# rensortino/DDP-Tutorial

Hardware: AMD Instinct MI355X
Metric: images/sec (whole node), ResNet-18 CIFAR-10 (higher is better)
Workload: dtype bf16; 1 GPU; model=resnet18, global_batch=8192, image_size=32, num_classes=10, parallelism=dp1, sync_bn=False, hip_graph=False

## Files before the change

mi355x/csrc/bindings.cpp:

```cpp
#include <torch/extension.h>

#include <tuple>
#include <vector>

at::Tensor relu_bwd(at::Tensor dy, at::Tensor y);
at::Tensor mfma_probe32(at::Tensor A, at::Tensor B);
void sgd_step(at::Tensor p, at::Tensor g, at::Tensor m, double lr, double mu,
              double wd, double gscale);
void grad_stats(at::Tensor g, at::Tensor slab, at::Tensor out);
void sgd_step_guarded(at::Tensor p, at::Tensor g, at::Tensor m,
                      at::Tensor state, c10::optional<at::Tensor> lr_dev,
                      double lr, double mu, double wd, double gscale,
                      double max_norm, c10::optional<at::Tensor> ema,
                      c10::optional<at::Tensor> clock);
void clock_advance(at::Tensor clock, c10::optional<at::Tensor> state,
                   at::Tensor table, double decay, bool warmup);
void scaler_update(at::Tensor state, double gscale, double max_norm,
                   double growth, double backoff, long interval);
void lars_stats(at::Tensor p, at::Tensor g, at::Tensor table, at::Tensor tens,
                at::Tensor slab, at::Tensor state, at::Tensor stats,
                double gscale, double max_norm, double wd, double eta,
                double eps);
void lars_step(at::Tensor p, at::Tensor g, at::Tensor m, at::Tensor table,
               at::Tensor tens, at::Tensor state, at::Tensor stats,
               c10::optional<at::Tensor> lr_dev, double lr, double mu,
               double wd, double gscale, double max_norm,
               c10::optional<at::Tensor> ema, c10::optional<at::Tensor> clock);
at::Tensor cast_to_16(at::Tensor src, at::Tensor like);
at::Tensor cast_permute_krsc(at::Tensor w, at::Tensor like);
at::Tensor cast_permute_krsc_pad(at::Tensor w, at::Tensor like);
at::Tensor cast_permute_rsck(at::Tensor w, at::Tensor like);

at::Tensor conv2d_fwd(at::Tensor x, at::Tensor w, at::Tensor bias,
                      long stride, long pad, long act, long kR, long kS);
at::Tensor conv2d_dgrad(at::Tensor dy, at::Tensor wflip, long stride,
                        long pad, long H, long W, at::Tensor addin);
at::Tensor conv2d_wgrad(at::Tensor x, at::Tensor dy, long R, long S,
                        long stride, long pad);
std::vector<at::Tensor> conv2d_fwd_stats(at::Tensor x, at::Tensor w,
                                         long stride, long pad, long kR,
                                         long kS);
std::vector<at::Tensor> conv2d_fwd_scaled(at::Tensor x, at::Tensor w,
                                          at::Tensor asc, at::Tensor ash,
                                          long stride, long pad,
                                          bool want_stats);
at::Tensor conv2d_wgrad_scaled(at::Tensor x, at::Tensor asc, at::Tensor ash,
                               at::Tensor dy, long R, long S, long stride,
                               long pad);

at::Tensor bn_stats(at::Tensor x);
at::Tensor bn_finalize(at::Tensor stats, at::Tensor running_mean,
                       at::Tensor running_var, double m_total,
                       double momentum, double eps);
std::vector<at::Tensor> bn_apply(at::Tensor x, at::Tensor mean, at::Tensor invstd,
                    at::Tensor gamma, at::Tensor beta, at::Tensor res,
                    long act, bool want_mask);
at::Tensor bn_bwd_reduce(at::Tensor x, at::Tensor dy, at::Tensor y,
                         at::Tensor mean, at::Tensor invstd,
                         at::Tensor mask, at::Tensor asc, at::Tensor ash);
std::vector<at::Tensor> bn_bwd_dx(at::Tensor x, at::Tensor dy, at::Tensor y,
                                  at::Tensor mean, at::Tensor invstd,
                                  at::Tensor gamma, at::Tensor dgamma,
                                  at::Tensor dbeta, double m_total,
                                  bool want_dres, at::Tensor mask,
                                  at::Tensor asc, at::Tensor ash);

std::vector<at::Tensor> maxpool_fwd(at::Tensor x, long kernel, long stride,
                                    long pad);
at::Tensor maxpool_bwd(at::Tensor dy, at::Tensor idx, long H, long W,
                       long kernel, long stride, long pad);
at::Tensor global_avg_pool(at::Tensor x);

at::Tensor linear_fwd(at::Tensor x, at::Tensor w, at::Tensor bias, long act);
at::Tensor linear_dgrad(at::Tensor dy, at::Tensor w, at::Tensor wt);
at::Tensor linear_wgrad(at::Tensor x, at::Tensor dy);
at::Tensor gemm_nt_mfma(at::Tensor A, at::Tensor B, at::Tensor bias, long act,
                        bool out32);

std::vector<at::Tensor> cross_entropy_fwd(at::Tensor logits,
                                          at::Tensor target);
at::Tensor cross_entropy_bwd(at::Tensor logits, at::Tensor target,
                             at::Tensor lse, at::Tensor dloss);
std::vector<at::Tensor> cross_entropy_soft_fwd(
    at::Tensor logits, at::Tensor y_a, c10::optional<at::Tensor> y_b,
    c10::optional<at::Tensor> lam, double eps);
at::Tensor cross_entropy_soft_bwd(at::Tensor logits, at::Tensor y_a,
                                  c10::optional<at::Tensor> y_b,
                                  c10::optional<at::Tensor> lam,
                                  at::Tensor lse, at::Tensor dloss,
                                  double eps);
void meter_update(at::Tensor state, at::Tensor slab, at::Tensor logits,
                  at::Tensor y_a, c10::optional<at::Tensor> y_b,
                  c10::optional<at::Tensor> lam, long k,
                  c10::optional<at::Tensor> loss,
                  c10::optional<at::Tensor> confusion, long pack);

std::tuple<at::Tensor, at::Tensor> gather_augment(
    at::Tensor data_u8, at::Tensor targets, at::Tensor indices,
    at::Tensor scale, at::Tensor shift, int64_t pad, bool flip, int64_t seed,
    int64_t epoch, at::Tensor like);
std::tuple<at::Tensor, at::Tensor, at::Tensor, at::Tensor> gather_augment_mix(
    at::Tensor data_u8, at::Tensor targets, at::Tensor indices,
    at::Tensor scale, at::Tensor shift, int64_t pad, bool flip, int64_t tc,
    int64_t tm, double inv_hw, int64_t seed, int64_t epoch, at::Tensor like);

void register_rccl(py::module_& m);

PYBIND11_MODULE(TORCH_EXTENSION_NAME, m) {
  register_rccl(m);
  m.def("relu_bwd", &relu_bwd);
  m.def("mfma_probe32", &mfma_probe32);
  m.def("sgd_step", &sgd_step);
  m.def("grad_stats", &grad_stats);
  m.def("sgd_step_guarded", &sgd_step_guarded);
  m.def("scaler_update", &scaler_update);
  m.def("clock_advance", &clock_advance);
  m.def("lars_stats", &lars_stats);
  m.def("lars_step", &lars_step);
  m.def("cast_to_16", &cast_to_16);
  m.def("cast_permute_krsc", &cast_permute_krsc);
  m.def("cast_permute_krsc_pad", &cast_permute_krsc_pad);
  m.def("cast_permute_rsck", &cast_permute_rsck);
  m.def("conv2d_fwd", &conv2d_fwd);
  m.def("conv2d_dgrad", &conv2d_dgrad);
  m.def("conv2d_wgrad", &conv2d_wgrad);
  m.def("conv2d_fwd_stats", &conv2d_fwd_stats);
  m.def("conv2d_fwd_scaled", &conv2d_fwd_scaled);
  m.def("conv2d_wgrad_scaled", &conv2d_wgrad_scaled);
  m.def("bn_stats", &bn_stats);
  m.def("bn_finalize", &bn_finalize);
  m.def("bn_apply", &bn_apply);
  m.def("bn_bwd_reduce", &bn_bwd_reduce);
  m.def("bn_bwd_dx", &bn_bwd_dx);
  m.def("maxpool_fwd", &maxpool_fwd);
  m.def("maxpool_bwd", &maxpool_bwd);
  m.def("global_avg_pool", &global_avg_pool);
  m.def("linear_fwd", &linear_fwd);
  m.def("linear_dgrad", &linear_dgrad);
  m.def("linear_wgrad", &linear_wgrad);
  m.def("gemm_nt_mfma", &gemm_nt_mfma);
  m.def("cross_entropy_fwd", &cross_entropy_fwd);
  m.def("cross_entropy_bwd", &cross_entropy_bwd);
  m.def("cross_entropy_soft_fwd", &cross_entropy_soft_fwd);
  m.def("cross_entropy_soft_bwd", &cross_entropy_soft_bwd);
  m.def("meter_update", &meter_update);
  m.def("gather_augment", &gather_augment);
  m.def("gather_augment_mix", &gather_augment_mix);
}
```

mi355x/csrc/bn.hip:

```cpp
#include "common.h"

namespace {

template <typename T16>
__global__ void bn_stats_kernel(const T16* __restrict__ x,
                                float* __restrict__ out,
                                long M, int C, long m_per_chunk) {
  const int c = blockIdx.y * blockDim.x + threadIdx.x;
  if (c >= C) return;
  const long m0 = (long)blockIdx.x * m_per_chunk;
  const long m1 = min(M, m0 + m_per_chunk);
  float s = 0.f, ss = 0.f;
  for (long m = m0; m < m1; ++m) {
    const float v = F16<T16>::to_f32(x[m * C + c]);
    s += v;
    ss += v * v;
  }
  float* o = out + (long)blockIdx.x * 2 * C;
  o[c] = s;
  o[C + c] = ss;
}

template <typename T16>
__global__ void bn_apply_kernel(const T16* __restrict__ x,
// ... 162 lines not shown
__global__ __launch_bounds__(256) void bn_apply_fast(
    const T16* __restrict__ x, const float* __restrict__ mean,
    const float* __restrict__ invstd, const float* __restrict__ gamma,
    const float* __restrict__ beta, const T16* __restrict__ res,
    T16* __restrict__ y, unsigned char* __restrict__ msk, long E, int C,
    int act) {
  const int c0 = ((blockIdx.x * blockDim.x + threadIdx.x) * 8) % C;
  float sc[8], sh[8];
#pragma unroll
  for (int u = 0; u < 8; ++u) {
    sc[u] = gamma[c0 + u] * invstd[c0 + u];
    sh[u] = beta[c0 + u] - mean[c0 + u] * sc[u];
  }
  const long stride = (long)gridDim.x * blockDim.x * 8;
  auto body = [&](long e) {
    const short8 vx = *reinterpret_cast<const short8*>(x + e);
    short8 vr = {};
    if (res) vr = *reinterpret_cast<const short8*>(res + e);
    short8 o;
    unsigned mb = 0;
#pragma unroll
    for (int u = 0; u < 8; ++u) {
      float v = s16_to_f32<T16>(vx[u]) * sc[u] + sh[u];
      if (res) v += s16_to_f32<T16>(vr[u]);
      if (act == 1) v = relu_f(v);
      o[u] = f32_to_s16<T16>(v);
      if (s16_to_f32<T16>(o[u]) > 0.f) mb |= 1u << u;
    }
    *reinterpret_cast<short8*>(y + e) = o;
    if (msk) msk[e >> 3] = (unsigned char)mb;
  };
  long e = (long)(blockIdx.x * blockDim.x + threadIdx.x) * 8;
  for (; e + stride < E; e += 2 * stride) {
    body(e);
    body(e + stride);
  }
  for (; e < E; e += stride) body(e);
}

template <typename T16, bool RC = false>
__global__ __launch_bounds__(256) void bn_bwd_dx_fast(
    const T16* __restrict__ x, const T16* __restrict__ dy,
    const unsigned char* __restrict__ msk, const float* __restrict__ mean,
    const float* __restrict__ invstd, const float* __restrict__ gamma,
    const float* __restrict__ dgamma, const float* __restrict__ dbeta,
    const float* __restrict__ asc, const float* __restrict__ ash,
    T16* __restrict__ dx, T16* __restrict__ dres, long E, int C,
    float inv_m) {
  const int c0 = ((blockIdx.x * blockDim.x + threadIdx.x) * 8) % C;
  float mu[8], is[8], g_[8], a_[8], b_[8], ac[8], ah[8];
#pragma unroll
  for (int u = 0; u < 8; ++u) {
    mu[u] = mean[c0 + u];
    is[u] = invstd[c0 + u];
    g_[u] = gamma[c0 + u] * is[u];
    a_[u] = dgamma[c0 + u] * inv_m;
    b_[u] = dbeta[c0 + u] * inv_m;
    if (RC) {
      ac[u] = asc[c0 + u];
      ah[u] = ash[c0 + u];
    }
  }
  const long stride = (long)gridDim.x * blockDim.x * 8;
  auto body = [&](long e) {
    const short8 vx = *reinterpret_cast<const short8*>(x + e);
    const short8 vd = *reinterpret_cast<const short8*>(dy + e);
    const unsigned mb = msk ? msk[e >> 3] : 0xffu;
    short8 odx, ods;
#pragma unroll
    for (int u = 0; u < 8; ++u) {
      float d = s16_to_f32<T16>(vd[u]);
      const float xv = s16_to_f32<T16>(vx[u]);
      if (RC) {
        if (xv * ac[u] + ah[u] <= 0.f) d = 0.f;
      } else if (!((mb >> u) & 1)) {
        d = 0.f;
      }
      if (dres) ods[u] = f32_to_s16<T16>(d);
      const float xh = (xv - mu[u]) * is[u];
      odx[u] = f32_to_s16<T16>(g_[u] * (d - b_[u] - xh * a_[u]));
    }
    *reinterpret_cast<short8*>(dx + e) = odx;
    if (dres) *reinterpret_cast<short8*>(dres + e) = ods;
  };
  long e = (long)(blockIdx.x * blockDim.x + threadIdx.x) * 8;
  for (; e + stride < E; e += 2 * stride) {
    body(e);
    body(e + stride);
  }
  for (; e < E; e += stride) body(e);
}

__global__ void bn_finalize_kernel(const float* __restrict__ stats,
                                   float* __restrict__ out,
                                   float* __restrict__ rmean,
                                   float* __restrict__ rvar, int C,
                                   float inv_m, float unbias, float momentum,
                                   float eps) {
  const int c = blockIdx.x * blockDim.x + threadIdx.x;
  if (c >= C) return;
  const float mean = stats[c] * inv_m;
  const float var = stats[C + c] * inv_m - mean * mean;
  out[c] = mean;
  out[C + c] = rsqrtf(var + eps);
  if (rmean) {
    rmean[c] = rmean[c] * (1.f - momentum) + mean * momentum;
    rvar[c] = rvar[c] * (1.f - momentum) + var * unbias * momentum;
  }
}

inline bool bn_fast_ok(long M, int C) {
  return C % 8 == 0 && 2048 % C == 0;
}

inline size_t bn_reduce_lds(int C) {
  const int rows = C > 512 ? 4 / (C / 512) : 4;
  return sizeof(float) * rows * 2 * C;
}

inline at::Tensor bn_partial_rows(const at::Tensor& x, unsigned nrows, int C) {
  return at::empty({(long)nrows, 2, C}, x.options().dtype(at::kFloat));
}

inline at::Tensor bn_fold(at::Tensor part, unsigned nrows, int C) {
  if (nrows == 1) return part.view({2, C});
  auto out = at::empty({2, C}, part.options());
  fold_rows(part, out, 2L * C, nrows);
  return out;
}

inline dim3 bn_fast_grid(long E, long& e_per_block) {
  static const long cap = EnvKnob("MI355X_BN_BLOCKS").num(512);
  long blocks = std::min<long>(cdiv_l(E, 2048), cap);
  e_per_block = cdiv_l(cdiv_l(E, blocks), 2048) * 2048;
  blocks = cdiv_l(E, e_per_block);
  return dim3((unsigned)blocks);
}

inline dim3 chan_grid(long M, int C, long& m_per_chunk, int block = 256) {
  const int cblocks = cdiv_i(C, block);
  long chunks = std::min<long>(cdiv_l(M, 1024), std::max(1, 2048 / cblocks));
  chunks = std::max<long>(chunks, 1);
  m_per_chunk = cdiv_l(M, chunks);
  return dim3((unsigned)chunks, cblocks);
}

inline int ew_grid2(long n, int block = 256) {
  return (int)std::min<long>(cdiv_l(n, block), 4096);
}

}

at::Tensor bn_finalize(at::Tensor stats, at::Tensor running_mean,
                       at::Tensor running_var, double m_total,
                       double momentum, double eps) {
  const int C = stats.size(1);
  auto out = at::empty_like(stats);
  const bool has_run = running_mean.numel() > 0;
  const double unbias = m_total / std::max(m_total - 1.0, 1.0);
  hipLaunchKernelGGL(bn_finalize_kernel, dim3(cdiv_i(C, 256)), dim3(256), 0,
                     cur_stream(), stats.data_ptr<float>(),
                     out.data_ptr<float>(),
                     has_run ? running_mean.data_ptr<float>() : nullptr,
                     has_run ? running_var.data_ptr<float>() : nullptr, C,
                     (float)(1.0 / m_total), (float)unbias, (float)momentum,
                     (float)eps);
// ... 105 lines not shown
                           mask.numel() ? mask.data_ptr<unsigned char>()
                                        : nullptr,
                           mean.data_ptr<float>(), invstd.data_ptr<float>(),
                           nullptr, nullptr,
                           out.data_ptr<float>(), E, C, e_per_block);
    });
    return bn_fold(out, grid.x, C);
  }
  long m_per_chunk;
  dim3 grid = chan_grid(M, C, m_per_chunk);
  auto out = bn_partial_rows(x, grid.x, C);
  DISPATCH_16(x, T16, {
    hipLaunchKernelGGL(bn_bwd_reduce_kernel<T16>, grid, dim3(256), 0,
                       cur_stream(), (const T16*)x.data_ptr(),
                       (const T16*)dy.data_ptr(),
                       y.numel() ? (const T16*)y.data_ptr() : nullptr,
                       mean.data_ptr<float>(),
                       invstd.data_ptr<float>(), out.data_ptr<float>(), M, C,
                       m_per_chunk);
  });
  return bn_fold(out, grid.x, C);
}

std::vector<at::Tensor> bn_bwd_dx(at::Tensor x, at::Tensor dy, at::Tensor y,
                                  at::Tensor mean, at::Tensor invstd,
                                  at::Tensor gamma, at::Tensor dgamma,
                                  at::Tensor dbeta, double m_total,
                                  bool want_dres, at::Tensor mask,
                                  at::Tensor asc, at::Tensor ash) {
  TORCH_CHECK(!(asc.defined() && asc.numel() > 0) ||
                  bn_fast_ok(x.numel() / x.size(-1), x.size(-1)),
              "mask recompute (asc/ash) needs the fast BN path");
  CHECK_GPU(x);
  CHECK_CONTIG(dy);
  const int C = x.size(-1);
  const long M = x.numel() / C;
  auto dx = at::empty_like(x);
  auto dres = want_dres ? at::empty_like(x) : at::Tensor();
  if (bn_fast_ok(M, C)) {
    const long E = M * (long)C;
    const int grid = (int)std::min<long>(cdiv_l(E, 256 * 8), 2048);
    const bool rc = asc.defined() && asc.numel() > 0;
    DISPATCH_16(x, T16, {
      if (rc)
        hipLaunchKernelGGL((bn_bwd_dx_fast<T16, true>), dim3(grid),
                           dim3(256), 0, cur_stream(),
                           (const T16*)x.data_ptr(),
                           (const T16*)dy.data_ptr(), nullptr,
                           mean.data_ptr<float>(), invstd.data_ptr<float>(),
                           gamma.data_ptr<float>(), dgamma.data_ptr<float>(),
                           dbeta.data_ptr<float>(), asc.data_ptr<float>(),
                           ash.data_ptr<float>(), (T16*)dx.data_ptr(),
                           want_dres ? (T16*)dres.data_ptr() : nullptr, E, C,
                           (float)(1.0 / m_total));
      else
        hipLaunchKernelGGL((bn_bwd_dx_fast<T16>), dim3(grid), dim3(256), 0,
                           cur_stream(), (const T16*)x.data_ptr(),
                           (const T16*)dy.data_ptr(),
                           mask.numel() ? mask.data_ptr<unsigned char>()
                                        : nullptr,
                           mean.data_ptr<float>(), invstd.data_ptr<float>(),
                           gamma.data_ptr<float>(), dgamma.data_ptr<float>(),
                           dbeta.data_ptr<float>(), nullptr, nullptr,
                           (T16*)dx.data_ptr(),
                           want_dres ? (T16*)dres.data_ptr() : nullptr, E, C,
                           (float)(1.0 / m_total));
    });
    return {dx, want_dres ? dres : at::Tensor()};
  }
  DISPATCH_16(x, T16, {
    hipLaunchKernelGGL(bn_bwd_dx_kernel<T16>, dim3(ew_grid2(M * C)),
                       dim3(256), 0, cur_stream(), (const T16*)x.data_ptr(),
                       (const T16*)dy.data_ptr(),
                       y.numel() ? (const T16*)y.data_ptr() : nullptr,
                       mean.data_ptr<float>(),
                       invstd.data_ptr<float>(), gamma.data_ptr<float>(),
                       dgamma.data_ptr<float>(), dbeta.data_ptr<float>(),
                       (T16*)dx.data_ptr(),
                       want_dres ? (T16*)dres.data_ptr() : nullptr, M, C,
                       (float)(1.0 / m_total));
  });
  return {dx, want_dres ? dres : at::Tensor()};
}
```

mi355x/models/layers.py:

```python

from __future__ import annotations

import math
import os

import torch
from torch import nn

from mi355x import ops


def to_model_layout(x: torch.Tensor) -> torch.Tensor:
    x = x.permute(0, 2, 3, 1)
    if x.is_cuda:
        x = x.to(ops.compute_dtype())
    return x.contiguous()


class Conv2d(nn.Module):

    def __init__(self, in_channels, out_channels, kernel_size, stride=1,
                 padding=0, bias=True, act=None, groups=1):
        super().__init__()
        if groups < 1 or in_channels % groups or out_channels % groups:
# ... 30 lines not shown
    def reset_parameters(self):
        nn.init.kaiming_uniform_(self.weight, a=math.sqrt(5))
        if self.bias is not None:
            bound = 1 / math.sqrt(self.weight.shape[1])
            nn.init.uniform_(self.bias, -bound, bound)

    def forward(self, x):
        return ops.linear(x, self.weight, self.bias, self.act)


class BatchNorm2d(nn.Module):

    def __init__(self, num_features, momentum=0.1, act=None):
        super().__init__()
        self.momentum, self.act = momentum, act
        self.weight = nn.Parameter(torch.ones(num_features))
        self.bias = nn.Parameter(torch.zeros(num_features))
        self.register_buffer("running_mean", torch.zeros(num_features))
        self.register_buffer("running_var", torch.ones(num_features))
        self._nbt = 0
        self.process_group = None

    @property
    def num_batches_tracked(self):
        return torch.tensor(self._nbt, dtype=torch.long)

    @num_batches_tracked.setter
    def num_batches_tracked(self, v):
        self._nbt = int(v)

    def _save_to_state_dict(self, destination, prefix, keep_vars):
        super()._save_to_state_dict(destination, prefix, keep_vars)
        destination[prefix + "num_batches_tracked"] = torch.tensor(
            self._nbt, dtype=torch.long)

    def _load_from_state_dict(self, state_dict, prefix, local_metadata,
                              strict, missing_keys, unexpected_keys,
                              error_msgs):
        key = prefix + "num_batches_tracked"
        if key in state_dict:
            self._nbt = int(state_dict[key])
        super()._load_from_state_dict(state_dict, prefix, local_metadata,
                                      strict, missing_keys, unexpected_keys,
                                      error_msgs)
        if key in unexpected_keys:
            unexpected_keys.remove(key)

    def forward(self, x, residual=None, stats=None):
        if self.training:
            self._nbt += 1
        return ops.batch_norm(x, self.weight, self.bias, self.running_mean,
                              self.running_var, self.training, self.momentum,
                              residual, self.act,
                              self.process_group if self.training else None,
                              stats)


def _fuse_stats():
    return os.environ.get("MI355X_FUSE_BN", "1") == "1"


def conv_bn(conv: "Conv2d", bn: "BatchNorm2d", x, residual=None):
    if (_fuse_stats() and x.is_cuda and bn.training and conv.bias is None
            and conv.act is None
            and (conv.weight.shape[1] % 64 == 0
                 or (conv.weight.shape[1] == 3
                     and ((conv.weight.shape[2] == 7 and conv.stride == 2)
                          or (conv.weight.shape[2] == 3
                              and conv.stride == 1))))):
        from mi355x.ops import functional as F_

        bn._nbt += 1

        y, stats = F_.conv2d_with_stats(x, conv.weight, conv.stride,
                                        conv.padding)
        if stats.numel() == 0:
            stats = None
        return ops.batch_norm(y, bn.weight, bn.bias, bn.running_mean,
                              bn.running_var, bn.training, bn.momentum,
                              residual, bn.act, bn.process_group, stats)
    return bn(conv(x), residual=residual)


def _tap_on():
    return os.environ.get("MI355X_TAP", "1") != "0"


def _lazy_mode():
    return os.environ.get("MI355X_LAZY_BN", "0")


def _lazy_ok(bn: "BatchNorm2d", conv: "Conv2d", x) -> bool:
    mode = _lazy_mode()
    if mode == "0":
        return False
    if mode == "g" and conv.weight.shape[2] != 1 and conv.stride == 1:
        return False
    C = conv.weight.shape[1]
    return (x.is_cuda and bn.training and bn.act == "relu"
            and conv.bias is None and conv.act is None
            and C % 64 == 0 and conv.weight.shape[0] % 64 == 0
            and 2048 % C == 0)


def bn_then_conv(bn: "BatchNorm2d", conv: "Conv2d", x, stats=None,
                 want_stats=False):
    if _lazy_ok(bn, conv, x) and x.requires_grad:
        return bn_conv_lazy(bn, conv, x, stats, want_stats)
    z = bn(x, stats=stats)
    if (want_stats and _fuse_stats() and z.is_cuda and bn.training
            and conv.bias is None and conv.act is None
            and conv.weight.shape[1] % 64 == 0):
        from mi355x.ops import functional as F_

        y, s2 = F_.conv2d_with_stats(z, conv.weight, conv.stride,
                                     conv.padding)
        if s2 is not None and s2.numel() == 0:
            s2 = None
        return y, s2
    return conv(z), None


def bn_conv_lazy(bn: "BatchNorm2d", conv: "Conv2d", x, stats=None,
                 want_stats=False):
    from mi355x.ops import functional as F_

    if bn.training:
        bn._nbt += 1
    out = F_.bn_conv(x, bn.weight, bn.bias, conv.weight, bn.running_mean,
                     bn.running_var, bn.momentum, stats,
                     bn.process_group if bn.training else None,
                     conv.stride, conv.padding, want_stats)
    if want_stats:
        y, s2 = out
        return y, (s2 if s2 is not None and s2.numel() else None)
    return out, None


def conv_bn_tap(conv: "Conv2d", bn: "BatchNorm2d", x, residual=None):
    if not (_tap_on() and x.is_cuda and conv.bias is None
            and conv.act is None):
        return conv_bn(conv, bn, x, residual=residual), x
    from mi355x.ops import functional as F_

    if _fuse_stats() and bn.training and conv.weight.shape[1] % 64 == 0:
        y, tap, stats = F_.conv2d_tap_stats(x, conv.weight, conv.stride,
                                            conv.padding)
        return bn(y, residual=residual, stats=stats), tap
    y, tap = F_.conv2d_tap(x, conv.weight, conv.stride, conv.padding)
    return bn(y, residual=residual), tap


class MaxPool2d(nn.Module):
    def __init__(self, kernel_size, stride=None, padding=0):
        super().__init__()
        self.kernel_size = kernel_size
        self.stride = stride or kernel_size
        self.padding = padding

    def forward(self, x):
        return ops.max_pool2d(x, self.kernel_size, self.stride, self.padding)
```

mi355x/models/resnet.py:

```python

from __future__ import annotations

import torch
from torch import nn

from .layers import (BatchNorm2d, Conv2d, Linear, MaxPool2d, _lazy_ok,
                     bn_conv_lazy, bn_then_conv, conv_bn, conv_bn_tap,
                     to_model_layout)
from mi355x import ops


class BasicBlock(nn.Module):
    expansion = 1

    def __init__(self, in_planes, planes, stride=1, downsample=None):
        super().__init__()
        self.conv1 = Conv2d(in_planes, planes, 3, stride, 1, bias=False)
        self.bn1 = BatchNorm2d(planes, act="relu")
        self.conv2 = Conv2d(planes, planes, 3, 1, 1, bias=False)
        self.bn2 = BatchNorm2d(planes, act="relu")
        self.downsample = downsample

    def forward(self, x):
        if _lazy_ok(self.bn1, self.conv2, x) and x.requires_grad:
            from mi355x.ops import functional as F_

            y1, tap, stats1 = F_.conv2d_tap_stats(
                x, self.conv1.weight, self.conv1.stride, self.conv1.padding)
            identity = (tap if self.downsample is None
                        else self.downsample(tap))
            y2, stats2 = bn_conv_lazy(self.bn1, self.conv2, y1, stats1,
                                      want_stats=True)
            return self.bn2(y2, residual=identity, stats=stats2)
        out, tap = conv_bn_tap(self.conv1, self.bn1, x)
        identity = tap if self.downsample is None else self.downsample(tap)
        out = conv_bn(self.conv2, self.bn2, out, residual=identity)
        return out


class Bottleneck(nn.Module):
    expansion = 4

    def __init__(self, in_planes, planes, stride=1, downsample=None):
        super().__init__()
        self.conv1 = Conv2d(in_planes, planes, 1, bias=False)
        self.bn1 = BatchNorm2d(planes, act="relu")
        self.conv2 = Conv2d(planes, planes, 3, stride, 1, bias=False)
        self.bn2 = BatchNorm2d(planes, act="relu")
        self.conv3 = Conv2d(planes, planes * 4, 1, bias=False)
        self.bn3 = BatchNorm2d(planes * 4, act="relu")
        self.downsample = downsample

    def forward(self, x):
        if x.is_cuda and x.requires_grad and self.bn1.training and (
                _lazy_ok(self.bn1, self.conv2, x)
                or _lazy_ok(self.bn2, self.conv3, x)):
            from mi355x.ops import functional as F_

            y1, tap, stats1 = F_.conv2d_tap_stats(
                x, self.conv1.weight, self.conv1.stride, self.conv1.padding)
            identity = (tap if self.downsample is None
                        else self.downsample(tap))
            y2, stats2 = bn_then_conv(self.bn1, self.conv2, y1, stats1,
                                      want_stats=True)
            y3, stats3 = bn_then_conv(self.bn2, self.conv3, y2, stats2,
                                      want_stats=True)
            return self.bn3(y3, residual=identity, stats=stats3)
        out, tap = conv_bn_tap(self.conv1, self.bn1, x)
        identity = tap if self.downsample is None else self.downsample(tap)
        out = conv_bn(self.conv2, self.bn2, out)
        out = conv_bn(self.conv3, self.bn3, out, residual=identity)
        return out


class Downsample(nn.Module):
    def __init__(self, in_planes, out_planes, stride):
        super().__init__()
        self.conv = Conv2d(in_planes, out_planes, 1, stride, bias=False)
        self.bn = BatchNorm2d(out_planes)

    def forward(self, x):
        return conv_bn(self.conv, self.bn, x)


class ResNet(nn.Module):
    def __init__(self, block, layers, num_classes=10, stem="cifar"):
        super().__init__()
        self.in_planes = 64
        if stem == "cifar":
            self.conv1 = Conv2d(3, 64, 3, 1, 1, bias=False)
            self.maxpool = None
        else:
            self.conv1 = Conv2d(3, 64, 7, 2, 3, bias=False)
            self.maxpool = MaxPool2d(3, 2, 1)
        self.bn1 = BatchNorm2d(64, act="relu")
        self.layer1 = self._make_layer(block, 64, layers[0], 1)
        self.layer2 = self._make_layer(block, 128, layers[1], 2)
        self.layer3 = self._make_layer(block, 256, layers[2], 2)
        self.layer4 = self._make_layer(block, 512, layers[3], 2)
        self.fc = Linear(512 * block.expansion, num_classes)
        for m in self.modules():
            if isinstance(m, Conv2d):
                nn.init.kaiming_normal_(m.weight, mode="fan_out",
                                        nonlinearity="relu")

    def _make_layer(self, block, planes, blocks, stride):
        downsample = None
        if stride != 1 or self.in_planes != planes * block.expansion:
            downsample = Downsample(self.in_planes, planes * block.expansion,
                                    stride)
        layers = [block(self.in_planes, planes, stride, downsample)]
        self.in_planes = planes * block.expansion
        layers += [block(self.in_planes, planes) for _ in range(1, blocks)]
        return nn.Sequential(*layers)

    def forward(self, x):
        x = to_model_layout(x)
        x = conv_bn(self.conv1, self.bn1, x)
        if self.maxpool is not None:
            x = self.maxpool(x)
        x = self.layer1(x)
        x = self.layer2(x)
        x = self.layer3(x)
        x = self.layer4(x)
        x = ops.global_avg_pool(x)
        return self.fc(x)


def resnet18(num_classes=10, stem="cifar"):
    return ResNet(BasicBlock, [2, 2, 2, 2], num_classes, stem)


def resnet50(num_classes=1000, stem="imagenet"):
    return ResNet(Bottleneck, [3, 4, 6, 3], num_classes, stem)
```

mi355x/ops/functional.py:

```python

from __future__ import annotations

from typing import NamedTuple

import numpy as np
import torch
import torch.nn.functional as F

from ._ext import ext

BN_EPS = 1e-5

_ACT_NONE = 0
_ACT_RELU = 1


def compute_dtype() -> torch.dtype:
    from mi355x import amp

    return amp.get_compute_dtype()



_cache_epoch = 0
# ... 325 lines not shown
        ctx.conf = (act, bias is not None)
        return y

    @staticmethod
    def backward(ctx, dy):
        x, w16, y = ctx.saved_tensors
        act, has_bias = ctx.conf
        dy = dy.contiguous()
        if act == _ACT_RELU:
            dy = _relu_mask_bwd(dy, y)
        dx = None
        if ctx.needs_input_grad[0]:
            wt = _w16_linear_t(ctx.weight_ref, dy.dtype)
            dx = ext().linear_dgrad(dy, w16, wt)
        dw = ext().linear_wgrad(x, dy) if ctx.needs_input_grad[1] else None
        db = dy.float().sum(dim=0) if (has_bias and ctx.needs_input_grad[2]) else None
        return dx, dw, db, None


def linear(x, weight, bias=None, act=None):
    a = _ACT_RELU if act == "relu" else _ACT_NONE
    if x.is_cuda:
        return _LinearFn.apply(x, weight, bias, a)
    y = F.linear(x, weight, bias)
    if a == _ACT_RELU:
        y = F.relu(y)
    return y




class _BNFn(torch.autograd.Function):

    @staticmethod
    def forward(ctx, x, gamma, beta, residual, running_mean, running_var,
                momentum, act, process_group, stats=None):
        N, H, W, C = x.shape
        m_local = N * H * W
        s = stats if stats is not None else ext().bn_stats(x)
        m_total = m_local
        if process_group is not None:
            import torch.distributed as dist

            dist.all_reduce(s, group=process_group)
            m_total = m_local * dist.get_world_size(process_group)
        empty = torch.empty(0, device=x.device)
        mi = ext().bn_finalize(
            s, running_mean if running_mean is not None else empty,
            running_var if running_var is not None else empty,
            float(m_total), momentum, BN_EPS)
        mean, invstd = mi[0], mi[1]
        res = residual if residual is not None else torch.empty(0, device=x.device, dtype=x.dtype)
        y, mask = ext().bn_apply(x, mean, invstd, gamma.detach().float(),
                                 beta.detach().float(), res, act, True)
        if mask is None:
            mask = torch.empty(0, device=x.device, dtype=torch.uint8)
        ctx.save_for_backward(x, y, mean, invstd, gamma, mask)
        ctx.conf = (act, residual is not None, m_total, process_group)
        return y

    @staticmethod
    def backward(ctx, dy):
        x, y, mean, invstd, gamma, mask = ctx.saved_tensors
        act, has_res, m_total, pg = ctx.conf
        dy = dy.contiguous()
        y_arg = y if act == _ACT_RELU else torch.empty(0, device=x.device,
                                                       dtype=x.dtype)
        ef = torch.empty(0, device=x.device)
        r = ext().bn_bwd_reduce(x, dy, y_arg, mean, invstd, mask, ef, ef)
        if pg is not None:
            import torch.distributed as dist

            dist.all_reduce(r, group=pg)
        dgamma, dbeta = r[0], r[1]
        want_dres = has_res and act == _ACT_RELU
        dx, dres = ext().bn_bwd_dx(x, dy, y_arg, mean, invstd,
                                   gamma.detach().float(), dgamma, dbeta,
                                   float(m_total), want_dres, mask, ef, ef)
        if has_res and not want_dres:
            dres = dy
        elif not has_res:
            dres = None
        return dx, dgamma, dbeta, dres, None, None, None, None, None, None


def batch_norm(x, gamma, beta, running_mean, running_var, training,
               momentum=0.1, residual=None, act=None, process_group=None,
               stats=None):
    a = _ACT_RELU if act == "relu" else _ACT_NONE
    if x.is_cuda:
        if training:
            return _BNFn.apply(x, gamma, beta, residual, running_mean,
                               running_var, momentum, a, process_group,
                               stats)
        mean = running_mean.float()
        invstd = torch.rsqrt(running_var.float() + BN_EPS)
        res = residual if residual is not None else torch.empty(0, device=x.device, dtype=x.dtype)
        return ext().bn_apply(x.contiguous(), mean, invstd,
                              gamma.detach().float(), beta.detach().float(),
                              res, a, False)[0]
    xc = x.permute(0, 3, 1, 2)
    y = F.batch_norm(xc, running_mean, running_var, gamma, beta, training,
                     momentum, BN_EPS).permute(0, 2, 3, 1)
    if residual is not None:
        y = y + residual
    if a == _ACT_RELU:
        y = F.relu(y)
    return y




class _MaxPoolFn(torch.autograd.Function):
    @staticmethod
    def forward(ctx, x, kernel, stride, padding):
        y, idx = ext().maxpool_fwd(x, kernel, stride, padding)
        ctx.save_for_backward(idx)
        ctx.conf = (x.shape, kernel, stride, padding)
        return y

    @staticmethod
    def backward(ctx, dy):
        (idx,) = ctx.saved_tensors
        xshape, kernel, stride, padding = ctx.conf
        dx = ext().maxpool_bwd(dy.contiguous(), idx, xshape[1], xshape[2],
                               kernel, stride, padding)
        return dx, None, None, None


def max_pool2d(x, kernel, stride=None, padding=0):
    stride = stride or kernel
    if x.is_cuda:
        return _MaxPoolFn.apply(x, kernel, stride, padding)
    y = F.max_pool2d(x.permute(0, 3, 1, 2), kernel, stride, padding)
    return y.permute(0, 2, 3, 1)


class _GAPFn(torch.autograd.Function):
    @staticmethod
    def forward(ctx, x):
        ctx.conf = x.shape
        return ext().global_avg_pool(x)

    @staticmethod
    def backward(ctx, dy):
        N, H, W, C = ctx.conf
        dx = (dy / (H * W)).reshape(N, 1, 1, C).expand(N, H, W, C).contiguous()
        return dx


def global_avg_pool(x):
    if x.is_cuda:
        return _GAPFn.apply(x)
    return x.mean(dim=(1, 2))




class _CEFn(torch.autograd.Function):
    @staticmethod
    def forward(ctx, logits, target):
        loss, lse = ext().cross_entropy_fwd(logits, target)
        ctx.save_for_backward(logits, target, lse)
        return loss

    @staticmethod
# ... 520 lines not shown
```

Baseline: 157,500 images/sec.

## Fuse downsample BN with main-branch BN, residual add and ReLU in one pass

Adds dual batch-norm kernels that normalize both the main conv output and the downsample conv output, add them, apply ReLU and emit a bit mask in one elementwise pass. The backward pass computes both branches' reductions and input gradients in shared passes. The goal is to avoid materializing the normalized downsample tensor and to cut separate full-tensor read/write passes in the three downsample blocks of ResNet-18. It is on by default, gated by an env flag, and relies on the fused-stats conv path and a specific channel layout.

```diff
diff --git a/mi355x/csrc/bindings.cpp b/mi355x/csrc/bindings.cpp
--- a/mi355x/csrc/bindings.cpp
+++ b/mi355x/csrc/bindings.cpp
@@ -64,6 +64,21 @@
                                   at::Tensor dbeta, double m_total,
                                   bool want_dres, at::Tensor mask,
                                   at::Tensor asc, at::Tensor ash);
+std::vector<at::Tensor> bn_apply_dual(at::Tensor x, at::Tensor mean,
+                                      at::Tensor invstd, at::Tensor gamma,
+                                      at::Tensor beta, at::Tensor xr,
+                                      at::Tensor mean_r, at::Tensor invstd_r,
+                                      at::Tensor gamma_r, at::Tensor beta_r);
+at::Tensor bn_bwd_reduce_dual(at::Tensor x, at::Tensor xr, at::Tensor dy,
+                              at::Tensor mask, at::Tensor mean,
+                              at::Tensor invstd, at::Tensor mean_r,
+                              at::Tensor invstd_r);
+std::vector<at::Tensor> bn_bwd_dx_dual(at::Tensor x, at::Tensor xr,
+                                       at::Tensor dy, at::Tensor mask,
+                                       at::Tensor mean, at::Tensor invstd,
+                                       at::Tensor gamma, at::Tensor mean_r,
+                                       at::Tensor invstd_r, at::Tensor gamma_r,
+                                       at::Tensor red, double m_total);
 
 std::vector<at::Tensor> maxpool_fwd(at::Tensor x, long kernel, long stride,
                                     long pad);
@@ -132,6 +147,9 @@
   m.def("bn_apply", &bn_apply);
   m.def("bn_bwd_reduce", &bn_bwd_reduce);
   m.def("bn_bwd_dx", &bn_bwd_dx);
+  m.def("bn_apply_dual", &bn_apply_dual);
+  m.def("bn_bwd_reduce_dual", &bn_bwd_reduce_dual);
+  m.def("bn_bwd_dx_dual", &bn_bwd_dx_dual);
   m.def("maxpool_fwd", &maxpool_fwd);
   m.def("maxpool_bwd", &maxpool_bwd);
   m.def("global_avg_pool", &global_avg_pool);
diff --git a/mi355x/csrc/bn.hip b/mi355x/csrc/bn.hip
--- a/mi355x/csrc/bn.hip
+++ b/mi355x/csrc/bn.hip
@@ -268,6 +268,176 @@
     }
     *reinterpret_cast<short8*>(dx + e) = odx;
     if (dres) *reinterpret_cast<short8*>(dres + e) = ods;
+  };
+  long e = (long)(blockIdx.x * blockDim.x + threadIdx.x) * 8;
+  for (; e + stride < E; e += 2 * stride) {
+    body(e);
+    body(e + stride);
+  }
+  for (; e < E; e += stride) body(e);
+}
+
+template <typename T16>
+__global__ __launch_bounds__(256) void bn_apply_dual_fast(
+    const T16* __restrict__ x, const T16* __restrict__ xr,
+    const float* __restrict__ mean, const float* __restrict__ invstd,
+    const float* __restrict__ gamma, const float* __restrict__ beta,
+    const float* __restrict__ mean_r, const float* __restrict__ invstd_r,
+    const float* __restrict__ gamma_r, const float* __restrict__ beta_r,
+    T16* __restrict__ y, unsigned char* __restrict__ msk, long E, int C) {
+  const int c0 = ((blockIdx.x * blockDim.x + threadIdx.x) * 8) % C;
+  float sc[8], sh[8], scr[8], shr[8];
+#pragma unroll
+  for (int u = 0; u < 8; ++u) {
+    sc[u] = gamma[c0 + u] * invstd[c0 + u];
+    sh[u] = beta[c0 + u] - mean[c0 + u] * sc[u];
+    scr[u] = gamma_r[c0 + u] * invstd_r[c0 + u];
+    shr[u] = beta_r[c0 + u] - mean_r[c0 + u] * scr[u];
+  }
+  const long stride = (long)gridDim.x * blockDim.x * 8;
+  auto body = [&](long e) {
+    const short8 vx = *reinterpret_cast<const short8*>(x + e);
+    const short8 vr = *reinterpret_cast<const short8*>(xr + e);
+    short8 o;
+    unsigned mb = 0;
+#pragma unroll
+    for (int u = 0; u < 8; ++u) {
+      float rf = s16_to_f32<T16>(vr[u]) * scr[u] + shr[u];
+      asm("" : "+v"(rf));
+      const float r = s16_to_f32<T16>(f32_to_s16<T16>(rf));
+      float v = s16_to_f32<T16>(vx[u]) * sc[u] + sh[u];
+      v += r;
+      v = relu_f(v);
+      o[u] = f32_to_s16<T16>(v);
+      if (s16_to_f32<T16>(o[u]) > 0.f) mb |= 1u << u;
+    }
+    *reinterpret_cast<short8*>(y + e) = o;
+    msk[e >> 3] = (unsigned char)mb;
+  };
+  long e = (long)(blockIdx.x * blockDim.x + threadIdx.x) * 8;
+  for (; e + stride < E; e += 2 * stride) {
+    body(e);
+    body(e + stride);
+  }
+  for (; e < E; e += stride) body(e);
+}
+
+template <typename T16>
+__global__ __launch_bounds__(256) void bn_reduce_dual_fast(
+    const T16* __restrict__ x, const T16* __restrict__ xr,
+    const T16* __restrict__ dy, const unsigned char* __restrict__ msk,
+    const float* __restrict__ mean, const float* __restrict__ invstd,
+    const float* __restrict__ mean_r, const float* __restrict__ invstd_r,
+    float* __restrict__ out,
+    long E, int C, long e_per_block) {
+  extern __shared__ __attribute__((aligned(16))) float lsum[];
+  const int tid = threadIdx.x;
+  const int c0 = (tid * 8) % C;
+  float s0[8] = {}, sr[8] = {}, s1[8] = {};
+  float mu[8], is[8], mur[8], isr[8];
+#pragma unroll
+  for (int u = 0; u < 8; ++u) {
+    mu[u] = mean[c0 + u];
+    is[u] = invstd[c0 + u];
+    mur[u] = mean_r[c0 + u];
+    isr[u] = invstd_r[c0 + u];
+  }
+  const long e0 = (long)blockIdx.x * e_per_block;
+  const long e1 = min(E, e0 + e_per_block);
+  constexpr long ESTEP = 256 * 8;
+  auto body = [&](long e) {
+    const short8 vx = *reinterpret_cast<const short8*>(x + e);
+    const short8 vr = *reinterpret_cast<const short8*>(xr + e);
+    const short8 vd = *reinterpret_cast<const short8*>(dy + e);
+    const unsigned mb = msk[e >> 3];
+#pragma unroll
+    for (int u = 0; u < 8; ++u) {
+      float d = s16_to_f32<T16>(vd[u]);
+      if (!((mb >> u) & 1)) d = 0.f;
+      const float xh = (s16_to_f32<T16>(vx[u]) - mu[u]) * is[u];
+      const float xhr = (s16_to_f32<T16>(vr[u]) - mur[u]) * isr[u];
+      s0[u] += d * xh;
+      sr[u] += d * xhr;
+      s1[u] += d;
+    }
+  };
+  long e = e0 + (long)tid * 8;
+  for (; e + 3 * ESTEP < e1; e += 4 * ESTEP) {
+#pragma unroll
+    for (int v = 0; v < 4; ++v) body(e + v * ESTEP);
+  }
+  for (; e < e1; e += ESTEP) body(e);
+  const int gstride = C / 8;
+  for (int off = 32; off >= gstride && off >= 1; off >>= 1) {
+#pragma unroll
+    for (int u = 0; u < 8; ++u) {
+      s0[u] += __shfl_xor(s0[u], off, kWave);
+      sr[u] += __shfl_xor(sr[u], off, kWave);
+      s1[u] += __shfl_xor(s1[u], off, kWave);
+    }
+  }
+  const bool leader = (threadIdx.x & 63) < gstride || gstride >= 64;
+  const int wpr = C > 512 ? C / 512 : 1;
+  const int rows = 4 / wpr;
+  const int row = (tid >> 6) / wpr;
+  if (leader) {
+#pragma unroll
+    for (int u = 0; u < 8; ++u) {
+      lsum[row * 3 * C + c0 + u] = s0[u];
+      lsum[row * 3 * C + C + c0 + u] = sr[u];
+      lsum[row * 3 * C + 2 * C + c0 + u] = s1[u];
+    }
+  }
+  __syncthreads();
+  float* o = out + (long)blockIdx.x * 3 * C;
+  for (int c = tid; c < 3 * C; c += 256) {
+    float a = lsum[c];
+    for (int r = 1; r < rows; ++r) a += lsum[r * 3 * C + c];
+    o[c] = a;
+  }
+}
+
+template <typename T16>
+__global__ __launch_bounds__(256) void bn_bwd_dx_dual_fast(
+    const T16* __restrict__ x, const T16* __restrict__ xr,
+    const T16* __restrict__ dy, const unsigned char* __restrict__ msk,
+    const float* __restrict__ mean, const float* __restrict__ invstd,
+    const float* __restrict__ gamma, const float* __restrict__ mean_r,
+    const float* __restrict__ invstd_r, const float* __restrict__ gamma_r,
+    const float* __restrict__ red,
+    T16* __restrict__ dx, T16* __restrict__ dxr, long E, int C, float inv_m) {
+  const int c0 = ((blockIdx.x * blockDim.x + threadIdx.x) * 8) % C;
+  float mu[8], is[8], g_[8], a_[8], mur[8], isr[8], gr[8], ar[8], b_[8];
+#pragma unroll
+  for (int u = 0; u < 8; ++u) {
+    mu[u] = mean[c0 + u];
+    is[u] = invstd[c0 + u];
+    g_[u] = gamma[c0 + u] * is[u];
+    a_[u] = red[c0 + u] * inv_m;
+    mur[u] = mean_r[c0 + u];
+    isr[u] = invstd_r[c0 + u];
+    gr[u] = gamma_r[c0 + u] * isr[u];
+    ar[u] = red[C + c0 + u] * inv_m;
+    b_[u] = red[2 * C + c0 + u] * inv_m;
+  }
+  const long stride = (long)gridDim.x * blockDim.x * 8;
+  auto body = [&](long e) {
+    const short8 vx = *reinterpret_cast<const short8*>(x + e);
+    const short8 vr = *reinterpret_cast<const short8*>(xr + e);
+    const short8 vd = *reinterpret_cast<const short8*>(dy + e);
+    const unsigned mb = msk[e >> 3];
+    short8 odx, odr;
+#pragma unroll
+    for (int u = 0; u < 8; ++u) {
+      float d = s16_to_f32<T16>(vd[u]);
+      if (!((mb >> u) & 1)) d = 0.f;
+      const float xh = (s16_to_f32<T16>(vx[u]) - mu[u]) * is[u];
+      const float xhr = (s16_to_f32<T16>(vr[u]) - mur[u]) * isr[u];
+      odx[u] = f32_to_s16<T16>(g_[u] * (d - b_[u] - xh * a_[u]));
+      odr[u] = f32_to_s16<T16>(gr[u] * (d - b_[u] - xhr * ar[u]));
+    }
+    *reinterpret_cast<short8*>(dx + e) = odx;
+    *reinterpret_cast<short8*>(dxr + e) = odr;
   };
   long e = (long)(blockIdx.x * blockDim.x + threadIdx.x) * 8;
   for (; e + stride < E; e += 2 * stride) {
@@ -539,3 +709,105 @@
   });
   return {dx, want_dres ? dres : at::Tensor()};
 }
+
+namespace {
+
+inline long bn_dual_check(const at::Tensor& x, const at::Tensor& xr) {
+  CHECK_GPU(x);
+  CHECK_CONTIG(x);
+  CHECK_CONTIG(xr);
+  CHECK_16BIT(x);
+  TORCH_CHECK(xr.scalar_type() == x.scalar_type() && xr.sizes() == x.sizes(),
+              "dual BN: the two inputs must agree in shape and dtype");
+  const int C = x.size(-1);
+  TORCH_CHECK(bn_fast_ok(x.numel() / C, C),
+              "dual BN needs the fast BN layout (C % 8 == 0, 2048 % C == 0)");
+  return x.numel();
+}
+
+inline const float* bn_vecC(const at::Tensor& v, int C) {
+  TORCH_CHECK(v.is_cuda() && v.scalar_type() == at::kFloat &&
+                  v.is_contiguous() && v.numel() == C,
+              "dual BN: per-channel operands are contiguous fp32 [C]");
+  return v.data_ptr<float>();
+}
+
+}
+
+std::vector<at::Tensor> bn_apply_dual(at::Tensor x, at::Tensor mean,
+                                      at::Tensor invstd, at::Tensor gamma,
+                                      at::Tensor beta, at::Tensor xr,
+                                      at::Tensor mean_r, at::Tensor invstd_r,
+                                      at::Tensor gamma_r, at::Tensor beta_r) {
+  const long E = bn_dual_check(x, xr);
+  const int C = x.size(-1);
+  auto y = at::empty_like(x);
+  auto mask = at::empty({E / 8}, x.options().dtype(at::kByte));
+  const int grid = (int)std::min<long>(cdiv_l(E, 256 * 8), 2048);
+  DISPATCH_16(x, T16, {
+    launch256(bn_apply_dual_fast<T16>, dim3(grid), 0, (const T16*)x.data_ptr(),
+              (const T16*)xr.data_ptr(), bn_vecC(mean, C), bn_vecC(invstd, C),
+              bn_vecC(gamma, C), bn_vecC(beta, C), bn_vecC(mean_r, C),
+              bn_vecC(invstd_r, C), bn_vecC(gamma_r, C), bn_vecC(beta_r, C),
+              (T16*)y.data_ptr(), mask.data_ptr<unsigned char>(), E, C);
+  });
+  return {y, mask};
+}
+
+at::Tensor bn_bwd_reduce_dual(at::Tensor x, at::Tensor xr, at::Tensor dy,
+                              at::Tensor mask, at::Tensor mean,
+                              at::Tensor invstd, at::Tensor mean_r,
+                              at::Tensor invstd_r) {
+  const long E = bn_dual_check(x, xr);
+  const int C = x.size(-1);
+  CHECK_CONTIG(dy);
+  TORCH_CHECK(dy.scalar_type() == x.scalar_type() && dy.numel() == E &&
+                  mask.is_cuda() && mask.scalar_type() == at::kByte &&
+                  mask.is_contiguous() && mask.numel() == E / 8,
+              "dual BN backward: dy like x, mask of one bit per element");
+  long e_per_block;
+  dim3 grid = bn_fast_grid(E, e_per_block);
+  auto part = at::empty({(long)grid.x, 3, C}, x.options().dtype(at::kFloat));
+  DISPATCH_16(x, T16, {
+    launch256(bn_reduce_dual_fast<T16>, grid, bn_reduce_lds(C) / 2 * 3,
+              (const T16*)x.data_ptr(), (const T16*)xr.data_ptr(),
+              (const T16*)dy.data_ptr(), mask.data_ptr<unsigned char>(),
+              bn_vecC(mean, C), bn_vecC(invstd, C), bn_vecC(mean_r, C),
+              bn_vecC(invstd_r, C), part.data_ptr<float>(), E, C, e_per_block);
+  });
+  if (grid.x == 1) return part.view({3, C});
+  auto out = at::empty({3, C}, part.options());
+  fold_rows(part, out, 3L * C, grid.x);
+  return out;
+}
+
+std::vector<at::Tensor> bn_bwd_dx_dual(at::Tensor x, at::Tensor xr,
+                                       at::Tensor dy, at::Tensor mask,
+                                       at::Tensor mean, at::Tensor invstd,
+                                       at::Tensor gamma, at::Tensor mean_r,
+                                       at::Tensor invstd_r, at::Tensor gamma_r,
+                                       at::Tensor red, double m_total) {
+  const long E = bn_dual_check(x, xr);
+  const int C = x.size(-1);
+  CHECK_CONTIG(dy);
+  TORCH_CHECK(dy.scalar_type() == x.scalar_type() && dy.numel() == E &&
+                  mask.is_cuda() && mask.scalar_type() == at::kByte &&
+                  mask.is_contiguous() && mask.numel() == E / 8,
+              "dual BN backward: dy like x, mask of one bit per element");
+  TORCH_CHECK(red.is_cuda() && red.scalar_type() == at::kFloat &&
+                  red.is_contiguous() && red.numel() == 3L * C,
+              "dual BN backward: red is contiguous fp32 [3,C]");
+  auto dx = at::empty_like(x);
+  auto dxr = at::empty_like(x);
+  const int grid = (int)std::min<long>(cdiv_l(E, 256 * 8), 2048);
+  DISPATCH_16(x, T16, {
+    launch256(bn_bwd_dx_dual_fast<T16>, dim3(grid), 0,
+              (const T16*)x.data_ptr(), (const T16*)xr.data_ptr(),
+              (const T16*)dy.data_ptr(), mask.data_ptr<unsigned char>(),
+              bn_vecC(mean, C), bn_vecC(invstd, C), bn_vecC(gamma, C),
+              bn_vecC(mean_r, C), bn_vecC(invstd_r, C), bn_vecC(gamma_r, C),
+              red.data_ptr<float>(), (T16*)dx.data_ptr(),
+              (T16*)dxr.data_ptr(), E, C, (float)(1.0 / m_total));
+  });
+  return {dx, dxr};
+}
diff --git a/mi355x/models/layers.py b/mi355x/models/layers.py
--- a/mi355x/models/layers.py
+++ b/mi355x/models/layers.py
@@ -136,6 +136,52 @@
     return bn(conv(x), residual=residual)
 
 
+def _bn_dual():
+    return os.environ.get("MI355X_BN_DUAL", "1") == "1"
+
+
+def _stats_conv_ok(conv: "Conv2d") -> bool:
+    return (conv.bias is None and conv.act is None and conv.groups == 1
+            and conv.weight.shape[1] % 64 == 0)
+
+
+def dual_ok(conv: "Conv2d", bn: "BatchNorm2d", down, x) -> bool:
+    if down is None or not (_bn_dual() and _fuse_stats()):
+        return False
+    C = bn.weight.shape[0]
+    return (x.is_cuda and bn.training and down.bn.training
+            and bn.act == "relu" and down.bn.act is None
+            and down.bn.weight.shape[0] == C and C % 8 == 0 and 2048 % C == 0
+            and _stats_conv_ok(conv) and _stats_conv_ok(down.conv)
+            and bn.process_group is down.bn.process_group)
+
+
+def conv_bn_dual(conv: "Conv2d", bn: "BatchNorm2d", x, down, tap):
+    from mi355x.ops import functional as F_
+
+    bn._nbt += 1
+    down.bn._nbt += 1
+    xr, stats_r = F_.conv2d_with_stats(tap, down.conv.weight,
+                                       down.conv.stride, down.conv.padding)
+    y, stats = F_.conv2d_with_stats(x, conv.weight, conv.stride,
+                                    conv.padding)
+    if stats.numel() and stats_r.numel() and y.shape == xr.shape:
+        return F_.batch_norm_dual(
+            y, bn.weight, bn.bias, bn.running_mean, bn.running_var,
+            bn.momentum, stats, xr, down.bn.weight, down.bn.bias,
+            down.bn.running_mean, down.bn.running_var, down.bn.momentum,
+            stats_r, bn.process_group)
+    identity = ops.batch_norm(xr, down.bn.weight, down.bn.bias,
+                              down.bn.running_mean, down.bn.running_var,
+                              True, down.bn.momentum, None, None,
+                              down.bn.process_group,
+                              stats_r if stats_r.numel() else None)
+    return ops.batch_norm(y, bn.weight, bn.bias, bn.running_mean,
+                          bn.running_var, True, bn.momentum, identity,
+                          bn.act, bn.process_group,
+                          stats if stats.numel() else None)
+
+
 def _tap_on():
     return os.environ.get("MI355X_TAP", "1") != "0"
 
diff --git a/mi355x/models/resnet.py b/mi355x/models/resnet.py
--- a/mi355x/models/resnet.py
+++ b/mi355x/models/resnet.py
@@ -5,8 +5,8 @@
 from torch import nn
 
 from .layers import (BatchNorm2d, Conv2d, Linear, MaxPool2d, _lazy_ok,
-                     bn_conv_lazy, bn_then_conv, conv_bn, conv_bn_tap,
-                     to_model_layout)
+                     bn_conv_lazy, bn_then_conv, conv_bn, conv_bn_dual,
+                     conv_bn_tap, dual_ok, to_model_layout)
 from mi355x import ops
 
 
@@ -33,6 +33,9 @@
                                       want_stats=True)
             return self.bn2(y2, residual=identity, stats=stats2)
         out, tap = conv_bn_tap(self.conv1, self.bn1, x)
+        if dual_ok(self.conv2, self.bn2, self.downsample, tap):
+            return conv_bn_dual(self.conv2, self.bn2, out, self.downsample,
+                                tap)
         identity = tap if self.downsample is None else self.downsample(tap)
         out = conv_bn(self.conv2, self.bn2, out, residual=identity)
         return out
@@ -67,6 +70,10 @@
                                       want_stats=True)
             return self.bn3(y3, residual=identity, stats=stats3)
         out, tap = conv_bn_tap(self.conv1, self.bn1, x)
+        if dual_ok(self.conv3, self.bn3, self.downsample, tap):
+            out = conv_bn(self.conv2, self.bn2, out)
+            return conv_bn_dual(self.conv3, self.bn3, out, self.downsample,
+                                tap)
         identity = tap if self.downsample is None else self.downsample(tap)
         out = conv_bn(self.conv2, self.bn2, out)
         out = conv_bn(self.conv3, self.bn3, out, residual=identity)
diff --git a/mi355x/ops/functional.py b/mi355x/ops/functional.py
--- a/mi355x/ops/functional.py
+++ b/mi355x/ops/functional.py
@@ -431,6 +431,59 @@
         elif not has_res:
             dres = None
         return dx, dgamma, dbeta, dres, None, None, None, None, None, None
+
+
+class _BNDualFn(torch.autograd.Function):
+
+    @staticmethod
+    def forward(ctx, x, gamma, beta, xr, gamma_r, beta_r, run, run_r,
+                momentum, momentum_r, process_group, stats, stats_r):
+        x, xr = x.contiguous(), xr.contiguous()
+        N, H, W, C = x.shape
+        m_total = N * H * W
+        if process_group is not None:
+            import torch.distributed as dist
+
+            dist.all_reduce(stats_r, group=process_group)
+            dist.all_reduce(stats, group=process_group)
+            m_total *= dist.get_world_size(process_group)
+        mi_r = ext().bn_finalize(stats_r, run_r[0], run_r[1], float(m_total),
+                                 momentum_r, BN_EPS)
+        mi = ext().bn_finalize(stats, run[0], run[1], float(m_total),
+                               momentum, BN_EPS)
+        y, mask = ext().bn_apply_dual(
+            x, mi[0], mi[1], gamma.detach().float(), beta.detach().float(),
+            xr, mi_r[0], mi_r[1], gamma_r.detach().float(),
+            beta_r.detach().float())
+        ctx.save_for_backward(x, xr, mi, mi_r, gamma, gamma_r, mask)
+        ctx.conf = (m_total, process_group)
+        return y
+
+    @staticmethod
+    def backward(ctx, dy):
+        x, xr, mi, mi_r, gamma, gamma_r, mask = ctx.saved_tensors
+        m_total, pg = ctx.conf
+        dy = dy.contiguous()
+        r = ext().bn_bwd_reduce_dual(x, xr, dy, mask, mi[0], mi[1], mi_r[0],
+                                     mi_r[1])
+        if pg is not None:
+            import torch.distributed as dist
+
+            dist.all_reduce(r, group=pg)
+        dx, dxr = ext().bn_bwd_dx_dual(
+            x, xr, dy, mask, mi[0], mi[1], gamma.detach().float(), mi_r[0],
+            mi_r[1], gamma_r.detach().float(), r, float(m_total))
+        return (dx, r[0], r[2], dxr, r[1], r[2].clone(), None, None, None,
+                None, None, None, None)
+
+
+def batch_norm_dual(x, gamma, beta, running_mean, running_var, momentum,
+                    stats, xr, gamma_r, beta_r, running_mean_r,
+                    running_var_r, momentum_r, stats_r, process_group=None):
+    return _BNDualFn.apply(x, gamma, beta, xr, gamma_r, beta_r,
+                           (running_mean, running_var),
+                           (running_mean_r, running_var_r), momentum,
+                           momentum_r, process_group, stats, stats_r)
 
 
 def batch_norm(x, gamma, beta, running_mean, running_var, training,
```

Measured after the change: 160,400 images/sec, median of 6. +1.9%, better.
